# spcl/gms

Hardware: AMD Instinct MI355X
Metric: edges-intersected/sec + achieved HBM GB/s, RMAT-26 triangle count @1/2/4/8 GPU (higher is better)
Workload: dtype int32 ids / uint64 counts

## Files before the change

### gms_amd/csrc/hip/device_graph.hip

```cpp
#include "device_graph.hpp"

#include <algorithm>
#include <mutex>
#include <array>
#include <chrono>
#include <cstdio>
#include <cstdlib>
#include <cstring>
#include <memory>
#include <new>
#include <random>

#include <rocprim/device/device_radix_sort.hpp>
#include <rocprim/device/device_scan.hpp>
#include <rocprim/device/device_segmented_radix_sort.hpp>
#include <rocprim/iterator/transform_iterator.hpp>

#include "../host/gmsx_internal.hpp"
#include "../host/tc_core_plan.hpp"
#include "kc4_mfma.hpp"

namespace gmsx {

Ctx &ctx() {
// ... 599 lines not shown
__global__ void k_ledge_fill(int64_t first, int64_t end, const int32_t *__restrict__ order, const int64_t *__restrict__ hoff, const int64_t *__restrict__ toff,
                             const int32_t *__restrict__ tadj, const int32_t *__restrict__ tsplit, const int32_t *__restrict__ dplus,
                             int32_t core, const int64_t *__restrict__ ebeg, int nparts, int part, uint4 *__restrict__ ledge) {
    const int64_t pos = first + int64_t(blockIdx.x) * blockDim.x + threadIdx.x;
    if (pos >= end) return;
    const int32_t u = order[pos];
    if (u < core) return;
    const int64_t hb = hoff[u], tb = toff[u];
    const int tl = int(toff[u + 1] - tb);
    const unsigned long long hu = (unsigned long long)hb | ((unsigned long long)(hoff[u + 1] - hb) << 40);
    int64_t e = ebeg[pos - first];
    for (int i = tsplit[u]; i < tl; ++i) {
        const int32_t v = tadj[tb + i];
        if (dplus[v] >= kHeavy) continue;
        if (nparts <= 1 || shard_of(e, nparts) == part) {
            const unsigned long long tu = (unsigned long long)tb | ((unsigned long long)i << 40);
            const unsigned long long hv = (unsigned long long)hoff[v] | ((unsigned long long)(hoff[v + 1] - hoff[v]) << 40);
            const unsigned long long tv = (unsigned long long)toff[v] | ((unsigned long long)(toff[v + 1] - toff[v]) << 40);
            const int64_t slot = nparts <= 1 ? e : e / nparts;
            ledge[2 * slot] = make_uint4(uint32_t(hu), uint32_t(hu >> 32), uint32_t(tu), uint32_t(tu >> 32));
            ledge[2 * slot + 1] = make_uint4(uint32_t(hv), uint32_t(hv >> 32), uint32_t(tv), uint32_t(tv >> 32));
        }
        ++e;
    }
}

__device__ __forceinline__ uint32_t cut_hub_units(const uint32_t *__restrict__ spool, unsigned long long d, int below, int32_t v) {
    const uint32_t units = uint32_t(d) & 0x3fffffu, form = (uint32_t(d) >> 22) & 3u;
    if (form == kFormList) return min(units, uint32_t(below + 7) / 8u);
    if (form == kFormBitset) return min(units, uint32_t(v + 127) / 128u);
    const uint4 *row = reinterpret_cast<const uint4 *>(spool) + (d >> 24);
    uint32_t lo = 0, hi = units;
    while (lo < hi) {
        const uint32_t mid = (lo + hi) >> 1;
        if (int32_t(row[mid].x & 0xffffu) < v) lo = mid + 1; else hi = mid;
    }
    return lo;
}
__device__ __forceinline__ uint32_t cut_tail_units(const uint32_t *__restrict__ tpool, unsigned long long d, int below, int32_t v) {
    const uint32_t units = uint32_t(d) & 0x3fffffu, form = (uint32_t(d) >> 22) & 3u;
    if (form != kFormDelta) return min(units, uint32_t(below + 3) / 4u);
    const uint4 *row = reinterpret_cast<const uint4 *>(tpool) + (d >> 24);
    uint32_t lo = 0, hi = units;
    while (lo < hi) {
        const uint32_t mid = (lo + hi) >> 1;
        if (int32_t(row[mid].x) < v) lo = mid + 1; else hi = mid;
// ... 160 lines not shown
        *p = nullptr;
        return GMSX_ERR_DEVICE_MEM;
    }
    if (hipMalloc(reinterpret_cast<void **>(p), bytes) != hipSuccess) {
        (void)hipGetLastError();
        *p = nullptr;
        return GMSX_ERR_DEVICE_MEM;
    }
    if (g) g->device_bytes += int64_t(bytes);
    return GMSX_OK;
}

struct DevGuard {
    void *p;
    ~DevGuard() { (void)hipFree(p); }
};

static void free_tc(gmsx_graph *g) {
    auto drop = [](auto *&p) {
        (void)hipFree(p);
        p = nullptr;
    };
    drop(g->tsplit); drop(g->srow); drop(g->srow2); drop(g->ksplit); drop(g->spool); drop(g->trow); drop(g->htask.lo); drop(g->htask.hi); drop(g->ttask.lo); drop(g->ttask.hi); drop(g->hitem); drop(g->titem); drop(g->tunits);
    drop(g->ledge); drop(g->tpool); drop(g->shard_hitem); drop(g->shard_titem); drop(g->core_bits);
    g->tc_core = 0;
    g->shard_idx_part = g->shard_idx_nparts = -1;
    g->device_bytes -= g->tc_bytes;
    g->tc_bytes = 0;
    g->tc_ready = false;
    g->htask_entries = g->ttask_entries = g->hitems = g->titems = g->inline_hentries = g->inline_tentries = 0;
    g->n_ledge = g->ledge_total = 0;
    g->task_reverse = g->inline_units = g->spool_units = g->tpool_units = 0;
    g->stats_part = g->stats_nparts = -1;
}

static void free_graph(gmsx_graph *g) {
    if (!g) return;
    (void)hipFree(g->off);
    (void)hipFree(g->adj);
    (void)hipFree(g->newid);
    (void)hipFree(g->oldid);
    (void)hipFree(g->hoff);
    (void)hipFree(g->hadj);
    (void)hipFree(g->toff);
    (void)hipFree(g->tadj);
    (void)hipFree(g->bmoff);
    (void)hipFree(g->bmpool);
    (void)hipFree(g->tsplit);
    (void)hipFree(g->srow);
    (void)hipFree(g->srow2);
    (void)hipFree(g->ksplit);
    (void)hipFree(g->spool);
    (void)hipFree(g->trow);
    (void)hipFree(g->htask.lo);
    (void)hipFree(g->htask.hi);
    (void)hipFree(g->ttask.lo);
    (void)hipFree(g->ttask.hi);
    (void)hipFree(g->hitem);
    (void)hipFree(g->titem);
    (void)hipFree(g->tunits);
    (void)hipFree(g->shard_hitem);
    (void)hipFree(g->shard_titem);
    (void)hipFree(g->ledge);
    (void)hipFree(g->core_bits);
    (void)hipFree(g->tpool);
    (void)hipFree(g->dplus);
    (void)hipFree(g->order);
    (void)hipFree(g->kc_rel);
    (void)hipFree(g->kc_aoff);
    (void)hipFree(g->kc_arena);
    (void)hipFree(g->kc_rec);
    (void)hipFree(g->kc_item);
    (void)hipFree(g->kc_relt);
    (void)hipFree(g->kc_rect);
    (void)hipFree(g->kc_itemt);
    (void)hipFree(g->scratch);
    (void)hipFree(g->acc);
    delete g;
}

int exclusive_scan_i64(const int64_t *in, int64_t *out, int64_t count, hipStream_t s) {
    size_t tmp_bytes = 0;
    GMSX_HIP(rocprim::exclusive_scan(nullptr, tmp_bytes, in, out, int64_t(0), size_t(count), rocprim::plus<int64_t>(), s));
    void *tmp = nullptr;
    GMSX_HIP(hipMalloc(&tmp, tmp_bytes ? tmp_bytes : 8));
    DevGuard g_tmp{tmp};
// ... 503 lines not shown
        inline_t_base = big_units + small_units;
        g->tpool_units = inline_t_base + inline_t_units;
        if (g->tpool_units >= (int64_t(1) << 40)) return GMSX_ERR_DEVICE_MEM;
        if (int rc = dmalloc(&g->trow, n, g)) return rc;
        if (int rc = dmalloc(&g->tpool, (g->tpool_units + kPoolSlack) * 4, g)) return rc;
        GMSX_HIP(hipMemsetD32Async(reinterpret_cast<hipDeviceptr_t>(g->tpool), int(0xFFFFFFFEu), size_t(g->tpool_units + kPoolSlack) * 4, s));
        if (n > 0)
            hipLaunchKernelGGL(k_trow_fill, dim3(unsigned((n + 255) / 256)), dim3(256), 0, s, n, g->toff, g->tadj, uoff, soff, real, form, g->trow, g->tpool);
        GMSX_HIP(hipStreamSynchronize(s));
    }

    pt.mark("tail stream rows");
    if (n_work > 0) {
        GMSX_HIP(hipMemsetAsync(inl_h, 0, size_t(n + 1) * sizeof(unsigned long long), s));
        GMSX_HIP(hipMemsetAsync(inl_t, 0, size_t(n + 1) * sizeof(unsigned long long), s));
        hipLaunchKernelGGL(k_inline_rows<true>, dim3(grid_for_waves(n_work)), dim3(256), 0, s, int64_t(0), n_work, g->order, g->hoff, g->hadj, g->toff,
                           g->tadj, g->dplus, g->inline_limit, g->inline_first, g->tc_core, opos, g->shard_nparts, g->shard_part, inl_h, inl_t, ihoff, itoff, inline_h_base, reinterpret_cast<uint16_t *>(g->spool),
                           inline_t_base, reinterpret_cast<int32_t *>(g->tpool));
    }
    pt.mark("inline rows fill");
    {
        const int64_t nl = n_work - n_heavy;
        g->n_ledge = g->ledge_total = 0;
        if (nl > 0) {
            int64_t *ecnt = nullptr, *ebeg = nullptr;
            if (int rc = dmalloc(&ecnt, nl + 1, nullptr)) return rc;
            DevGuard g_ec{ecnt};
            if (int rc = dmalloc(&ebeg, nl + 1, nullptr)) return rc;
            DevGuard g_eb{ebeg};
            hipLaunchKernelGGL(k_ledge_count, dim3(unsigned(nl / 256 + 1)), dim3(256), 0, s, n_heavy, n_work, g->order, g->toff, g->tadj, g->tsplit, g->dplus, g->tc_core, ecnt);
            if (int rc = exclusive_scan_i64(ecnt, ebeg, nl + 1, s)) return rc;
            GMSX_HIP(hipMemcpy(&g->ledge_total, ebeg + nl, sizeof(int64_t), hipMemcpyDeviceToHost));
            const int np = g->shard_nparts > 1 ? g->shard_nparts : 1, pp = g->shard_nparts > 1 ? g->shard_part : 0;
            {
                const int64_t full = g->ledge_total / np, rem = g->ledge_total % np;
                g->n_ledge = np <= 1 ? g->ledge_total : full + (((full & 1) ? np - 1 - pp : pp) < rem ? 1 : 0);
            }
            if (int rc = dmalloc(&g->ledge, 2 * g->n_ledge + 2, g)) return rc;
            hipLaunchKernelGGL(k_ledge_fill, dim3(unsigned(nl / 256 + 1)), dim3(256), 0, s, n_heavy, n_work, g->order, g->hoff, g->toff, g->tadj, g->tsplit, g->dplus, g->tc_core, ebeg,
                               np, pp, g->ledge);
            GMSX_HIP(hipStreamSynchronize(s));
        }
    }
    pt.mark("light pivot list");
    {
        int two_sided = 1;
        if (const char *e = opt("TC_TWO_SIDED")) two_sided = std::atoi(e) != 0;
// ... 404 lines not shown
```

### gms_amd/csrc/hip/device_graph.hpp

```cpp
#pragma once
#include <hip/hip_runtime.h>

#include <cstdint>

#include "gmsx.h"
#include "gmsx_internal.hpp"

#if !defined(GMSX_DEV_HOOKS) &&                                                                                                               \
    (defined(GMSX_KC_NO_PROBE) || defined(GMSX_KC_NO_HITS) || defined(GMSX_KC_NO_TAIL) || defined(GMSX_KC_NO_INNER) || defined(GMSX_KC_CELLS_ONLY) ||   \
     defined(GMSX_KC_NO_ROWS) || defined(GMSX_KC_BUILD_ONLY) || defined(GMSX_KC_NO_SLAB_CALL) || defined(GMSX_KC_NO_PAIRS) || defined(GMSX_KC_SLAB_ROW_SCAN) || \
     defined(GMSX_BK_AB) || defined(GMSX_BK_NO_HIT_ATOMICS) || defined(GMSX_BK_STATS) || defined(GMSX_TC_NO_PROBE) || defined(GMSX_TC_STAGING_ONLY))
#error "A/B switches need -DGMSX_DEV_HOOKS (tools/ab_lib.sh sets it); the default build of libgmsx.so carries none of them"
#endif

struct __attribute__((aligned(64))) gmsx_tc_item {
    uint64_t bc;
    uint64_t cont;
    int32_t pivot;
    int32_t pos;
    uint32_t kind;
    uint16_t fbeg[4];
    uint32_t reserved[7];
};
static_assert(sizeof(gmsx_tc_item) == 64, "work item record = one 64-byte line");
// ... 27 lines not shown
    int32_t *tadj = nullptr;
    int64_t *bmoff = nullptr;
    uint32_t *bmpool = nullptr;
    int32_t dense_limit = 0;
    int32_t bitset_limit = 0;
    unsigned long long *srow = nullptr;
    unsigned long long *srow2 = nullptr;
    int32_t *ksplit = nullptr;
    uint32_t *spool = nullptr;
    int64_t spool_units = 0;
    TaskList htask{nullptr, nullptr, false};
    TaskList ttask{nullptr, nullptr, true};
    int64_t htask_entries = 0, ttask_entries = 0;
    struct gmsx_tc_item *hitem = nullptr, *titem = nullptr;
    int64_t hitems = 0, titems = 0;
    int64_t inline_hentries = 0, inline_tentries = 0;
    mutable struct gmsx_tc_item *shard_hitem = nullptr, *shard_titem = nullptr;
    mutable int64_t shard_hitems = 0, shard_titems = 0;
    mutable int shard_idx_part = -1, shard_idx_nparts = -1;
    int32_t *tunits = nullptr;
    int64_t task_reverse = 0;
    uint4 *ledge = nullptr;
    int64_t n_ledge = 0, ledge_total = 0;
    uint32_t *core_bits = nullptr;
    int32_t tc_core = 0;
    mutable int core_bytes_k = -1, core_bytes_part = -1, core_bytes_nparts = -1;
    mutable uint64_t core_bytes = 0;
    int tc_hot_windows = 0;
    uint32_t tc_window_units = 1;
    int tc_hot_min = 0;
    int inline_first = 64;
    int32_t inline_limit = 0;
    int64_t inline_units = 0;
    unsigned long long *trow = nullptr;
    uint32_t *tpool = nullptr;
    int64_t tpool_units = 0;
    int32_t *tsplit = nullptr;
    int64_t dense_rows = 0, bmpool_words = 0;
    bool rows_sorted = false;
    int32_t *dplus = nullptr;
    int32_t *order = nullptr;
    int64_t hub_entries = 0, tail_entries = 0;
    int32_t max_dplus = 0;
    int32_t max_deg = 0;
    mutable bool kc_rev_tried = false;
    mutable uint32_t *kc_rel = nullptr;
// ... 59 lines not shown
__host__ __device__ inline int tail_class(const TcClasses &cc, unsigned long long d) {
    return cc.tail_base() + (((uint32_t(d) >> 22) & 3u) == 2u ? kLenClasses : 0) + length_class(uint32_t(d) & 0x3fffffu);
}
__host__ __device__ inline void hub_phase_range(const TcClasses &cc, const uint32_t *c, int64_t len, int ph, int64_t *b, int64_t *e) {
    int64_t start = 0;
    for (int q = 0;; ++q) {
        const int64_t end = q < cc.hot_windows ? int64_t(c[(q + 1) * kHubClasses]) : len;
        const bool own = q == cc.hot_windows || end - start >= cc.hot_min;
        if (q == ph) {
            *b = start;
            *e = own ? end : start;
            return;
        }
        if (own) start = end;
    }
}
__host__ __device__ inline int shard_of(int64_t pos, int nparts) {
    const int j = int(pos % nparts);
    return ((pos / nparts) & 1) ? nparts - 1 - j : j;
}
static constexpr int kHeavy = 64;
static constexpr int kDeltaIds = 14;

__host__ __device__ inline int64_t bitset_words(int32_t v) { return ((int64_t(v) + 31) / 32 + 3) & ~int64_t(3); }

struct Ctx {
    int device = -1;
    hipStream_t stream = nullptr;
    hipStream_t own_stream = nullptr;
    hipEvent_t ev[4] = {nullptr, nullptr, nullptr, nullptr};
    hipStream_t side[2] = {nullptr, nullptr};
    hipEvent_t ev_fork = nullptr, ev_join[2] = {nullptr, nullptr};
    int compute_units = 0;
};
Ctx &ctx();
int ensure_init();
int kclique_vertex_counts(const gmsx_graph *g, unsigned long long *d_counts, gmsx_stats *st);
int count_dplus_ge(const gmsx_graph *g, int32_t threshold, int64_t *out);
int exclusive_scan_i64(const int64_t *in, int64_t *out, int64_t count, hipStream_t s);
int ensure_tc(const gmsx_graph *g);
int ensure_tc_shard(const gmsx_graph *g, int part, int nparts);
int tc_shard_items(const gmsx_graph *g, int part, int nparts);
int tc_vertex_counts_device(const gmsx_graph *g, unsigned long long *d_counts, gmsx_stats *st);
int tc_full_partial(const gmsx_graph *g, int part, int nparts, uint64_t *partial, gmsx_stats *st);

__device__ __forceinline__ int uni32(int x) { return __builtin_amdgcn_readfirstlane(x); }
// ... 19 lines not shown
```

### gms_amd/csrc/hip/tc.hip

```cpp
#include "device_graph.hpp"
#include "kc4_mfma.hpp"
#include "../host/tc_core_plan.hpp"

#include <algorithm>
#include <type_traits>
#include <rocprim/device/device_radix_sort.hpp>
#include <rocprim/device/device_reduce.hpp>
#include <rocprim/device/device_reduce_by_key.hpp>
#include <cstdio>
#include <cstdlib>
#include <cstring>

namespace gmsx {

static constexpr int kAccSlots = 64;
static constexpr int kAccStride = 16;

struct __attribute__((packed, aligned(4))) u4u { uint32_t x, y, z, w; };

__device__ __forceinline__ int64_t readlane64(int64_t x, int l) {
    const uint32_t lo = __builtin_amdgcn_readlane(uint32_t(uint64_t(x)), l);
    const uint32_t hi = __builtin_amdgcn_readlane(uint32_t(uint64_t(x) >> 32), l);
    return int64_t((uint64_t(hi) << 32) | lo);
}
// ... 614 lines not shown
            for (int ka = 0; ka < 4; ++ka) {
                if (ka >= nat) break;
                const int ia = sub + 16 * ka;
                const uint32_t a = ia < tlu ? rows.at[ka] : 0xFFFFFFFFu;
                bool m = false;
#pragma unroll
                for (int kb = 0; kb < 4; ++kb) {
                    if (kb >= nbt) break;
                    const int ib = sub + 16 * kb;
                    const uint32_t x = ib < tlv ? rows.bt[kb] : 0xFFFFFFFEu;
                    m |= row_has(a, x);
                }
                c += m ? 1u : 0u;
            }
            total += c;
            rec = rec_n;
            rows = rows_n;
            rec_n = rec_nn;
        }
    }
    block_add(total, red, lane, wave, tid, acc);
}

__global__ __launch_bounds__(1024) void k_tc_core(const uint32_t *__restrict__ bits, int WS, int K, int nb, int nblk, int part, int nparts,
                                                  unsigned long long *__restrict__ acc) {
    __shared__ unsigned long long red[16];
    auto lane_id = [] { return int(__builtin_amdgcn_mbcnt_hi(~0u, __builtin_amdgcn_mbcnt_lo(~0u, 0u))); };
    const int wave = uni32(int(threadIdx.x) >> 6);
    const int x = blockIdx.x & 7, y = blockIdx.x >> 3, Y = int(gridDim.x) >> 3;
    const int Q = 16 * Y, q = y * 16 + wave;
    const int ns = (nblk - part + nparts - 1) / nparts;
    uint32_t cnt = 0;
    for (int j = 0;; ++j) {
        const int sidx = (8 * j + ((j & 1) ? 7 - x : x)) * Q + q;
        if (sidx >= ns) break;
        const int t = sidx * nparts + part;
        int c = int((__builtin_sqrtf(8.0f * float(t) + 1.0f) - 1.0f) * 0.5f);
        while (c * (c + 1) / 2 > t) --c;
        while ((c + 1) * (c + 2) / 2 <= t) ++c;
        const int bj = nb - 1 - c, bi = bj + (t - c * (c + 1) / 2);
        int lane = lane_id();
        asm volatile("" : "+v"(lane));
        cnt += Kc4mBlock<2>::run(bits, WS, K, bi, bj, lane);
    }
    const int lane = lane_id();
    unsigned long long total = cnt;
    for (int sft = 32; sft > 0; sft >>= 1) total += __shfl_down(total, sft);
    if (lane == 0) red[wave] = total;
    __syncthreads();
    if (wave == 0 && lane == 0) {
        unsigned long long t = 0;
        for (int w = 0; w < 16; ++w) t += red[w];
        if (t) atomicAdd(&acc[(blockIdx.x & (kAccSlots - 1)) * kAccStride], t);
    }
}

__global__ __launch_bounds__(256) void k_tc_stats(const int64_t *__restrict__ hoff, const uint16_t *__restrict__ hadj,
                                                  const int64_t *__restrict__ toff, const int32_t *__restrict__ tadj,
                                                  const int32_t *__restrict__ dplus, const int32_t *__restrict__ order,
                                                  const int32_t *__restrict__ tunits, int32_t inline_limit, int inline_first, int32_t core, int64_t end, int nparts, int part,
                                                  unsigned long long *__restrict__ out) {
    const int lane = threadIdx.x & 63;
    const int64_t wave0 = (int64_t(blockIdx.x) * blockDim.x + threadIdx.x) >> 6;
    const int64_t nwaves = (int64_t(gridDim.x) * blockDim.x) >> 6;
    unsigned long long units = 0, probes = 0, bytes = 0;
    for (int64_t pos = wave0; pos < end; pos += nwaves) {
        if (nparts > 1 && shard_of(pos, nparts) != part) continue;
        const int32_t u = order[pos];
        const int du = dplus[u];
        if (du >= kHeavy) {
            if (lane == 0) units += (unsigned long long)tunits[pos];
            if (u < core) {
                if (lane == 0) units += (unsigned long long)du;
                continue;
            }
            const int hl = min(int(hoff[u + 1] - hoff[u]), inline_first), tl = min(int(toff[u + 1] - toff[u]), inline_first - hl);
            int32_t v = -1;
            if (lane < hl) {
                const uint32_t x = hadj[hoff[u] + lane];
                if (x != 0xFFFFu) v = int32_t(x);
            } else if (lane - hl < tl) v = tadj[toff[u] + lane - hl];
            if (v >= 0 && lane > 0 && (v < inline_limit || dplus[v] >= kHeavy)) ++units;
            continue;
        }
        const int hl = int(hoff[u + 1] - hoff[u]);
        if (lane == 0) units += (unsigned long long)du;
        if (du < 2 || u < core) continue;
        for (int64_t j = toff[u] + lane; j < toff[u + 1]; j += 64) {
            const int32_t v = tadj[j];
            if (v < inline_limit || dplus[v] >= kHeavy) continue;
            const unsigned long long hv = (unsigned long long)(hoff[v + 1] - hoff[v]), tv = (unsigned long long)(toff[v + 1] - toff[v]);
            bytes += 32ull + 2ull * hl + 4ull * (unsigned long long)(j - toff[u]) + 2ull * hv + 4ull * tv;
            probes += hv + tv;
        }
    }
    for (int s = 32; s > 0; s >>= 1) {
        units += __shfl_down(units, s);
        probes += __shfl_down(probes, s);
        bytes += __shfl_down(bytes, s);
    }
    if (lane == 0) {
        if (units) atomicAdd(&out[0], units);
        if (probes) atomicAdd(&out[1], probes);
        if (bytes) atomicAdd(&out[2], bytes);
    }
}
__global__ __launch_bounds__(256) void k_tc_item_stats(const int64_t *__restrict__ coff, int bytes_per_id, int tail, const TaskList task,
                                                       const gmsx_tc_item *__restrict__ items, int64_t n_items, int nparts, int part,
                                                       unsigned long long *__restrict__ out) {
    const int lane = threadIdx.x & 63;
    const int64_t wave0 = (int64_t(blockIdx.x) * blockDim.x + threadIdx.x) >> 6;
    const int64_t nwaves = (int64_t(gridDim.x) * blockDim.x) >> 6;
    unsigned long long probes = 0, bytes = 0;
    auto slots = [tail](unsigned long long d) -> unsigned long long {
        const unsigned long long n = d & 0x3fffffull, f = (d >> 22) & 3ull;
// ... 1 lines not shown
    };
    for (int64_t q = wave0; q < n_items; q += nwaves) {
        const gmsx_tc_item &it = items[q];
        if (nparts > 1 && shard_of(it.pos, nparts) != part) continue;
        const int ne = int(it.bc >> 40);
        const int64_t b = int64_t(it.bc & 0xffffffffffull);
        if (lane == 0) bytes += (unsigned long long)bytes_per_id * (unsigned long long)(coff[it.pivot + 1] - coff[it.pivot]);
        for (int i = lane; i < ne; i += 64) {
            const unsigned long long d = task.get(b + i);
            bytes += 6ull + 16ull * (d & 0x3fffffull);
            probes += slots(d);
        }
    }
    for (int s = 32; s > 0; s >>= 1) {
        probes += __shfl_down(probes, s);
        bytes += __shfl_down(bytes, s);
    }
    if (lane == 0) {
        if (probes) atomicAdd(&out[1], probes);
        if (bytes) atomicAdd(&out[2], bytes);
    }
}

__global__ __launch_bounds__(256) void k_tc_breakdown(const int64_t *__restrict__ hoff, const int64_t *__restrict__ toff, const int32_t *__restrict__ tadj,
                                                      const int32_t *__restrict__ dplus, const int32_t *__restrict__ order,
                                                      const TaskList htask, const gmsx_tc_item *__restrict__ hitem, int64_t hitems,
                                                      const TaskList ttask, const gmsx_tc_item *__restrict__ titem, int64_t titems,
                                                      int32_t inline_limit, int32_t core, int64_t first_light, int64_t end_light,
                                                      unsigned long long *__restrict__ out) {
    const int lane = threadIdx.x & 63;
    const int64_t wave0 = (int64_t(blockIdx.x) * blockDim.x + threadIdx.x) >> 6;
    const int64_t nwaves = (int64_t(gridDim.x) * blockDim.x) >> 6;
    unsigned long long c[15] = {0, 0, 0, 0, 0, 0, 0, 0, 0, 0, 0, 0, 0, 0, 0};
    for (int64_t q = wave0; q < hitems + titems; q += nwaves) {
        const bool tail = q >= hitems;
        const gmsx_tc_item &it = tail ? titem[q - hitems] : hitem[q];
        const TaskList task = tail ? ttask : htask;
        const int ne = int(it.bc >> 40);
        const int64_t b0 = int64_t(it.bc & 0xffffffffffull);
        if (lane == 0) {
            c[6] += tail ? 4ull * (unsigned long long)(toff[it.pivot + 1] - toff[it.pivot]) : 2ull * (unsigned long long)(hoff[it.pivot + 1] - hoff[it.pivot]);
            c[11] += (unsigned long long)ne;
            c[13] += 1;
        }
        for (int i = lane; i < ne; i += 64) {
            const unsigned long long d = task.get(b0 + i);
            const unsigned long long db = 16ull * (d & 0x3fffffull);
            const int fd = int((d >> 22) & 3);
            if (tail) c[fd == kFormDelta ? 4 : 3] += db;
            else c[fd == kFormList ? 0 : fd == kFormBitset ? 1 : 2] += db;
            c[5] += 6;
        }
    }
    for (int64_t pos = first_light + wave0; pos < end_light; pos += nwaves) {
        const int32_t u = order[pos];
        if (u < core) continue;
        const int64_t tb0 = toff[u], te = toff[u + 1];
        const unsigned long long hl = (unsigned long long)(hoff[u + 1] - hoff[u]);
        for (int64_t j = tb0 + lane; j < te; j += 64) {
            const int32_t v = tadj[j];
            if (v < inline_limit || dplus[v] >= kHeavy) continue;
            c[8] += 2ull * (unsigned long long)(hoff[v + 1] - hoff[v]);
            c[9] += 4ull * (unsigned long long)(toff[v + 1] - toff[v]);
            c[10] += 32ull + 2ull * hl + 4ull * (unsigned long long)(j - tb0);
            c[14] += 1;
        }
    }
    for (int k = 0; k < 15; ++k) {
        unsigned long long x = c[k];
        for (int s = 32; s > 0; s >>= 1) x += __shfl_down(x, s);
        if (lane == 0 && x) atomicAdd(&out[k], x);
    }
}

__device__ __forceinline__ int hist_bin(unsigned long long units) {
    if (units <= 16) return int(units) - 1;
    int b = 16;
    for (unsigned long long lim = 32; units > lim && b < 23; lim <<= 1) ++b;
    return b;
}
__global__ __launch_bounds__(256) void k_tc_comember_keys(const TaskList htask, const gmsx_tc_item *__restrict__ hitem, int64_t hitems, int batch,
                                                         unsigned long long *__restrict__ keys, uint32_t *__restrict__ vals, unsigned long long *__restrict__ sums) {
    unsigned long long ents = 0, units = 0;
    for (int64_t i = blockIdx.x; i < hitems; i += gridDim.x) {
        const gmsx_tc_item it = hitem[i];
        const unsigned long long first = it.bc & 0xffffffffffull;
        const int n = int(it.bc >> 40);
        const unsigned long long b = (unsigned long long)(it.pos / batch) << 40;
// ... 169 lines not shown
    const char *only = std::getenv("GMSX_TC_ONLY");
    if (only) {
        if (std::strcmp(only, "hub") != 0) n_hitems = 0;
        if (std::strcmp(only, "tail") != 0) n_titems = 0;
    }
#else
    const char *only = nullptr;
#endif
    Ctx &c = ctx();
    hipStream_t s = c.stream;
    unsigned long long *acc = g->acc;
    static_assert(kAccSlots * kAccStride + 16 <= kAccWords, "gmsx_graph::acc too small");
    unsigned int *qhead = reinterpret_cast<unsigned int *>(acc + kAccSlots * kAccStride + 4);
    static_assert((kQueueStride + 1) * sizeof(unsigned int) <= 12 * sizeof(unsigned long long), "queue heads past gmsx_graph::acc");
    GMSX_HIP(hipEventRecord(c.ev[0], s));
    GMSX_HIP(hipMemsetAsync(acc, 0, sizeof(unsigned long long) * kAccWords, s));
    GMSX_HIP(hipEventRecord(c.ev[1], s));

    int launches = 0;
    const int cus = c.compute_units > 0 ? c.compute_units : 256;
    const int64_t cap_blocks = int64_t(cus) * 16;
    const bool run_light = !only || std::strcmp(only, "light") == 0;
    const bool strided = nparts > 1 && g->shard_nparts == 1;
    const int64_t cnt_light = [&]() -> int64_t {
        if (!run_light) return 0;
        if (!strided) return g->n_ledge;
        const int64_t full = g->n_ledge / nparts, rem = g->n_ledge % nparts;
        return full + (((full & 1) ? nparts - 1 - part : part) < rem ? 1 : 0);
    }();
    const int overlap = [] { const char *e = opt("TC_OVERLAP"); return e ? std::atoi(e) : 0; }();
    const int persist = [] { const char *e = opt("TC_PERSIST"); return e ? std::atoi(e) : 1; }();
    const bool sides = overlap && c.side[0] && c.side[1];
    struct Join {
        Ctx &c;
        hipStream_t s;
        bool armed[2] = {false, false};
        ~Join() {
            for (int i = 0; i < 2; ++i)
                if (armed[i] && hipEventRecord(c.ev_join[i], c.side[i]) == hipSuccess) (void)hipStreamWaitEvent(s, c.ev_join[i], 0);
        }
    } join{c, s};
    const bool side_light = sides && cnt_light > 0 && n_hitems + n_titems > 0;
    const bool side_tail = sides && !persist && n_hitems > 0 && n_titems > 0;
    if (side_light || side_tail) GMSX_HIP(hipEventRecord(c.ev_fork, s));
    if (side_tail) {
        GMSX_HIP(hipStreamWaitEvent(c.side[0], c.ev_fork, 0));
        join.armed[0] = true;
    }
    if (side_light) {
        GMSX_HIP(hipStreamWaitEvent(c.side[1], c.ev_fork, 0));
        join.armed[1] = true;
    }
// ... 11 lines not shown
        const int wgs_env = [] { const char *e = opt("TC_ITEM_WGS"); return e ? std::atoi(e) : 0; }();
        auto grid = [&](int64_t n, int wgs) {
            return unsigned(std::max<int64_t>(1, std::min<int64_t>((n + kGrab - 1) / kGrab, int64_t(cus) * (wgs_env > 0 ? wgs_env : wgs))));
        };
        if (n_hitems > 0) {
            hipLaunchKernelGGL(k_tc_items<false>, dim3(grid(n_hitems, GMSX_TC_HUB_MIN_WAVES)), dim3(256), 0, s, g->hadj, g->tadj, g->spool, g->htask, hitem, int(n_hitems), qhead, acc);
            ++launches;
        }
        if (n_titems > 0) {
            hipLaunchKernelGGL(k_tc_items<true>, dim3(grid(n_titems, GMSX_TC_TAIL_MIN_WAVES)), dim3(256), 0, s, g->hadj, g->tadj, g->tpool, g->ttask, titem, int(n_titems),
                               qhead + kQueueStride, acc);
            ++launches;
        }
    } else {
        if (n_hitems > 0) {
            hipLaunchKernelGGL(k_tc_block, dim3(unsigned(n_hitems)), dim3(256), 0, s, g->hoff, g->hadj, g->spool, g->htask, hitem, acc);
            ++launches;
        }
        if (n_titems > 0) {
            hipLaunchKernelGGL(k_tc_tail, dim3(unsigned(n_titems)), dim3(256), 0, side_tail ? c.side[0] : s, g->toff, g->tadj, g->tpool, g->ttask, titem, acc);
            ++launches;
        }
    }
    if (cnt_light > 0) {
        const int64_t blocks = std::min<int64_t>((cnt_light + 15) / 16, int64_t(cus) * 8);
        hipLaunchKernelGGL(k_tc_light, dim3(unsigned(blocks)), dim3(256), 0, side_light ? c.side[1] : s, g->hadj, g->tadj, g->ledge, strided ? nparts : 1,
                           strided ? part : 0, cnt_light, acc);
        ++launches;
    }
    for (int i = 0; i < 2; ++i)
        if (join.armed[i]) {
            join.armed[i] = false;
            GMSX_HIP(hipEventRecord(c.ev_join[i], c.side[i]));
            GMSX_HIP(hipStreamWaitEvent(s, c.ev_join[i], 0));
        }
    GMSX_HIP(hipEventRecord(c.ev[2], s));
    GMSX_HIP(hipGetLastError());

    const bool need_stats = st && !(g->stats_part == part && g->stats_nparts == nparts);
    if (need_stats) {
        if (g->n > 0) {
            const int64_t blocks = std::min<int64_t>((g->n + 3) / 4, cap_blocks);
            hipLaunchKernelGGL(k_tc_stats, dim3(unsigned(blocks)), dim3(256), 0, s, g->hoff, g->hadj, g->toff, g->tadj, g->dplus, g->order,
                               g->tunits, g->inline_limit, g->inline_first, g->tc_core, g->n, nparts, part, acc + kAccSlots * kAccStride);
        }
        if (g->hitems > 0)
            hipLaunchKernelGGL(k_tc_item_stats, dim3(unsigned(std::min<int64_t>((g->hitems + 3) / 4, cap_blocks))), dim3(256), 0, s, g->hoff, 2, 0, g->htask, g->hitem,
                               g->hitems, nparts, part, acc + kAccSlots * kAccStride);
        if (g->titems > 0)
            hipLaunchKernelGGL(k_tc_item_stats, dim3(unsigned(std::min<int64_t>((g->titems + 3) / 4, cap_blocks))), dim3(256), 0, s, g->toff, 4, 1, g->ttask, g->titem,
                               g->titems, nparts, part, acc + kAccSlots * kAccStride);
    }
    unsigned long long host[kAccSlots * kAccStride + 3];
    GMSX_HIP(hipMemcpyAsync(host, acc, sizeof(host), hipMemcpyDeviceToHost, s));
    GMSX_HIP(hipStreamSynchronize(s));
    unsigned long long total = 0;
    for (int i = 0; i < kAccSlots; ++i) total += host[i * kAccStride];
    *partial = total;
    if (st) {
        float ms_setup = 0.f, ms_kernel = 0.f;
        GMSX_HIP(hipEventElapsedTime(&ms_setup, c.ev[0], c.ev[1]));
        GMSX_HIP(hipEventElapsedTime(&ms_kernel, c.ev[1], c.ev[2]));
        st->kernel_ms = ms_kernel;
        st->setup_ms = ms_setup;
        if (need_stats) {
            g->stats_part = part;
            g->stats_nparts = nparts;
// ... 15 lines not shown

using namespace gmsx;

extern "C" {

int gmsx_tc_divisor(int algo) { return algo == GMSX_TC_FULL ? 3 : 1; }

int gmsx_tc_stream_breakdown(const gmsx_graph *g, uint64_t *out21) {
    return gmsx::guard([&]() -> int {
        if (!g || !out21) return GMSX_ERR_INVALID;
        if (int rc = ensure_init()) return rc;
        if (int rc = ensure_tc(g)) return rc;
        hipStream_t s = ctx().stream;
        std::memset(out21, 0, 21 * sizeof(uint64_t));
        if (g->n == 0) return GMSX_OK;
        int64_t n_block = 0, n_work = 0;
        if (int rc = count_dplus_ge(g, kHeavy, &n_block)) return rc;
        if (int rc = count_dplus_ge(g, 2, &n_work)) return rc;
        unsigned long long *acc = nullptr;
        GMSX_HIP(hipMalloc(reinterpret_cast<void **>(&acc), 21 * 8));
        struct Guard { void *p; ~Guard() { (void)hipFree(p); } } g1{acc};
        GMSX_HIP(hipMemsetAsync(acc, 0, 21 * 8, s));
        const int cus = ctx().compute_units > 0 ? ctx().compute_units : 256;
        hipLaunchKernelGGL(k_tc_breakdown, dim3(unsigned(cus * 16)), dim3(256), 0, s, g->hoff, g->toff, g->tadj, g->dplus, g->order, g->htask,
                           g->hitem, g->hitems, g->ttask, g->titem, g->titems, g->inline_limit, g->tc_core, n_block, n_work, acc);
        GMSX_HIP(hipMemcpyAsync(out21, acc, 21 * 8, hipMemcpyDeviceToHost, s));
        GMSX_HIP(hipStreamSynchronize(s));
        GMSX_HIP(hipGetLastError());
        out21[7] = uint64_t(g->inline_units) * 16ull;
        out21[12] = uint64_t(g->inline_hentries + g->inline_tentries);
        out21[15] = core_bytes_of(g, 0, 1);
        out21[16] = uint64_t(g->tc_core);
        return GMSX_OK;
    });
}

int gmsx_tc_row_histogram(const gmsx_graph *g, uint64_t *out256) {
    return gmsx::guard([&]() -> int {
        uint64_t *out248 = out256;
        if (!g || !out248) return GMSX_ERR_INVALID;
        if (int rc = ensure_init()) return rc;
        if (int rc = ensure_tc(g)) return rc;
        hipStream_t s = ctx().stream;
        std::memset(out248, 0, 256 * sizeof(uint64_t));
        if (g->n == 0) return GMSX_OK;
        unsigned long long *acc = nullptr;
        GMSX_HIP(hipMalloc(reinterpret_cast<void **>(&acc), 256 * 8));
        struct Guard { void *p; ~Guard() { (void)hipFree(p); } } g1{acc};
// ... 90 lines not shown
```

### gms_amd/csrc/host/loader.cpp

```cpp
#include "gmsx_internal.hpp"

#include <fcntl.h>
#include <sys/mman.h>
#include <sys/stat.h>
#include <unistd.h>

#include <algorithm>
#ifdef _OPENMP
#include <parallel/algorithm>
#endif
#include <atomic>
#include <cerrno>
#include <cmath>
#include <cstdio>
#include <cstdlib>
#include <cstring>
#include <ctime>
#include <fstream>
#include <limits>
#include <memory>
#include <new>
#include <random>
#include <sstream>
#include <string>
// ... 631 lines not shown
void parallel_memcpy(void *dst, const void *src, size_t bytes) {
#ifdef _OPENMP
#pragma omp parallel
    {
        const size_t nt = size_t(omp_get_num_threads()), t = size_t(omp_get_thread_num());
        const size_t per = ((bytes + nt - 1) / nt + 4095) & ~size_t(4095), lo = std::min(bytes, per * t), hi = std::min(bytes, lo + per);
        if (hi > lo) std::memcpy(static_cast<char *>(dst) + lo, static_cast<const char *>(src) + lo, hi - lo);
    }
#else
    std::memcpy(dst, src, bytes);
#endif
}
namespace {
struct Option {
    const char *name;
    char value[32];
    bool set;
};
Option g_options[] = {
    {"TIMING", "", false}, {"MEM_TRACE", "", false}, {"BK_VERBOSE", "", false},
    {"INLINE_LIMIT", "", false}, {"TC_INLINE_FIRST", "", false}, {"TC_DELTA", "", false}, {"TC_DELTA_PCT", "", false}, {"TC_GAP12", "", false},
    {"TC_HYBRID", "", false}, {"TC_TAIL_DELTA", "", false}, {"TC_TWO_SIDED", "", false}, {"TC_HOT_WINDOWS", "", false}, {"TC_HOT_KB", "", false},
    {"TC_HOT_MIN", "", false}, {"TC_TEST_MAX_UNITS", "", false}, {"TC_KEEP_ROWS", "", false}, {"TC_MEM_LIMIT_MB", "", false}, {"TC_OVERLAP", "", false},
    {"TC_PERSIST", "", false}, {"TC_ITEM_WGS", "", false}, {"TC_CORE", "", false}, {"SORT_CHUNK", "", false}, {"UPLOAD_STAGED", "", false}, {"INIT_LAZY", "", false},
    {"KC_SLAB_MB", "", false}, {"KC_MAXD", "", false}, {"KC_STREAMS", "", false}, {"KC_PIPE_ALL", "", false}, {"KC_STREAM_BUILD", "", false},
    {"KC_REVERSE", "", false}, {"KC_REV_MIN", "", false}, {"KC_REV_FACTOR", "", false}, {"KC_REV_TAIL", "", false}, {"KC_REV_TAIL_MIN", "", false}, {"KC_REV_GW", "", false}, {"KC_TRI", "", false}, {"KC_MFMA", "", false}, {"KC_POOL_MB", "", false},
    {"BK_MAXC", "", false}, {"BK_ARENA_MB", "", false}, {"BK_GROUPS", "", false}, {"BK_SMALL_P", "", false}, {"BK_SMALL_P_GROUPS", "", false},
    {"BK_BUDGET", "", false}, {"BK_BUDGET0", "", false}, {"BK_RESUME_GRAB", "", false}, {"BK_SPLIT_BUILD", "", false}, {"BK_TINY_ROOTS", "", false},
    {"BK_TINY_BESIDE", "", false},
    {"BK_LIST_ARENA_MB", "", false},
    {"KCSTAR_SLAB_MB", "", false},
    {"CORE_WG_FRONTIER", "", false},
    {"COLOR_WG_FRONTIER", "", false},
    {"TRUSS_WG_FRONTIER", "", false},
    {"LP_LDS_MAXN", "", false}, {"LP_SLAB_MB", "", false},
};
Option *find_option(const char *name) {
    if (!name) return nullptr;
    for (Option &o : g_options)
        if (std::strcmp(o.name, name) == 0) return &o;
    return nullptr;
}
}

const char *opt(const char *name) {
    const Option *o = find_option(name);
    return o && o->set ? o->value : nullptr;
// ... 242 lines not shown
```

Before: 16.10 billion.

## Pack light edge pairs into contiguous size-classed blocks for triangle counting

Replaces the indirect light-edge descriptors (offsets into hub and tail adjacency pools) with pre-materialised, padded blocks that hold both endpoints' hub and tail id lists, grouped into six size classes. A new templated kernel per class streams each block with coalesced loads into LDS and does fixed-depth branchless binary searches, prefetching the next block while it computes. This targets scattered gathers and variable-length loops in the light path. In exchange it costs extra preprocessing, duplicated adjacency storage with padding overhead, and six launches instead of one.

```diff
diff --git a/gms_amd/csrc/hip/device_graph.hip b/gms_amd/csrc/hip/device_graph.hip
--- a/gms_amd/csrc/hip/device_graph.hip
+++ b/gms_amd/csrc/hip/device_graph.hip
@@ -645,6 +645,84 @@
             ledge[2 * slot + 1] = make_uint4(uint32_t(hv), uint32_t(hv >> 32), uint32_t(tv), uint32_t(tv >> 32));
         }
         ++e;
+    }
+}
+
+__global__ void k_lpack_count(int64_t first, int64_t end, const int32_t *__restrict__ order, const int64_t *__restrict__ hoff, const uint16_t *__restrict__ hadj,
+                              const int64_t *__restrict__ toff, const int32_t *__restrict__ tadj, const int32_t *__restrict__ tsplit, const int32_t *__restrict__ dplus,
+                              int32_t core, int64_t *__restrict__ cnt) {
+    const int64_t p = int64_t(blockIdx.x) * blockDim.x + threadIdx.x, nl = end - first;
+    if (p >= nl) return;
+    int64_t c[kLightClasses];
+#pragma unroll
+    for (int k = 0; k < kLightClasses; ++k) c[k] = 0;
+    const int32_t u = order[first + p];
+    if (u >= core) {
+        const int64_t tb = toff[u];
+        const int tl = int(toff[u + 1] - tb), ah = light_hub_ids(hoff, hadj, u);
+        for (int i = tsplit[u]; i < tl; ++i) {
+            const int32_t v = tadj[tb + i];
+            if (dplus[v] >= kHeavy) continue;
+            const int cls = light_class(ah, i, light_hub_ids(hoff, hadj, v), int(toff[v + 1] - toff[v]));
+#pragma unroll
+            for (int k = 0; k < kLightClasses; ++k) c[k] += cls == k ? 1 : 0;
+        }
+    }
+#pragma unroll
+    for (int k = 0; k < kLightClasses; ++k) cnt[int64_t(k) * nl + p] = c[k];
+}
+struct LpackPlan {
+    int64_t class_beg[kLightClasses];
+    int64_t unit_base[kLightClasses];
+};
+__device__ __forceinline__ uint4 lpack_hub_unit(const uint16_t *__restrict__ row, int len, int q) {
+    uint32_t w[4];
+#pragma unroll
+    for (int j = 0; j < 4; ++j) {
+        const int i = 8 * q + 2 * j;
+        const uint32_t lo = i < len ? row[i] : 0xFFFFu, hi = i + 1 < len ? row[i + 1] : 0xFFFFu;
+        w[j] = lo | (hi << 16);
+    }
+    return make_uint4(w[0], w[1], w[2], w[3]);
+}
+__device__ __forceinline__ uint4 lpack_tail_unit(const int32_t *__restrict__ row, int len, int q, uint32_t filler) {
+    uint32_t w[4];
+#pragma unroll
+    for (int j = 0; j < 4; ++j) w[j] = 4 * q + j < len ? uint32_t(row[4 * q + j]) : filler;
+    return make_uint4(w[0], w[1], w[2], w[3]);
+}
+__global__ void k_lpack_fill(int64_t first, int64_t end, const int32_t *__restrict__ order, const int64_t *__restrict__ hoff, const uint16_t *__restrict__ hadj,
+                             const int64_t *__restrict__ toff, const int32_t *__restrict__ tadj, const int32_t *__restrict__ tsplit, const int32_t *__restrict__ dplus,
+                             int32_t core, const int64_t *__restrict__ beg, const LpackPlan plan, int nparts, int part, uint4 *__restrict__ lpack) {
+    const int64_t p = int64_t(blockIdx.x) * blockDim.x + threadIdx.x, nl = end - first;
+    if (p >= nl) return;
+    const int32_t u = order[first + p];
+    if (u < core) return;
+    int64_t next[kLightClasses];
+#pragma unroll
+    for (int k = 0; k < kLightClasses; ++k) next[k] = beg[int64_t(k) * nl + p] - plan.class_beg[k];
+    const int64_t hb = hoff[u], tb = toff[u];
+    const int tl = int(toff[u + 1] - tb), ah = light_hub_ids(hoff, hadj, u);
+    for (int i = tsplit[u]; i < tl; ++i) {
+        const int32_t v = tadj[tb + i];
+        if (dplus[v] >= kHeavy) continue;
+        const int64_t hv = hoff[v], tv = toff[v];
+        const int bh = light_hub_ids(hoff, hadj, v), bt = int(toff[v + 1] - tv);
+        const int cls = light_class(ah, i, bh, bt);
+        int64_t k = 0, base = 0;
+#pragma unroll
+        for (int c = 0; c < kLightClasses; ++c)
+            if (cls == c) {
+                k = next[c]++;
+                base = plan.unit_base[c];
+            }
+        if (nparts > 1 && shard_of(k, nparts) != part) continue;
+        const LightShape sh = light_shape(cls);
+        uint4 *blk = lpack + base + (nparts <= 1 ? k : k / nparts) * sh.stride();
+        for (int q = 0; q < sh.ah; ++q) *blk++ = lpack_hub_unit(hadj + hb, ah, q);
+        for (int q = 0; q < sh.at; ++q) *blk++ = lpack_tail_unit(tadj + tb, i, q, 0xFFFFFFFFu);
+        for (int q = 0; q < sh.bh; ++q) *blk++ = lpack_hub_unit(hadj + hv, bh, q);
+        for (int q = 0; q < sh.bt; ++q) *blk++ = lpack_tail_unit(tadj + tv, bt, q, 0xFFFFFFFEu);
     }
 }
 
@@ -851,7 +929,7 @@
         p = nullptr;
     };
     drop(g->tsplit); drop(g->srow); drop(g->srow2); drop(g->ksplit); drop(g->spool); drop(g->trow); drop(g->htask.lo); drop(g->htask.hi); drop(g->ttask.lo); drop(g->ttask.hi); drop(g->hitem); drop(g->titem); drop(g->tunits);
-    drop(g->ledge); drop(g->tpool); drop(g->shard_hitem); drop(g->shard_titem); drop(g->core_bits);
+    drop(g->ledge); drop(g->lpack); drop(g->tpool); drop(g->shard_hitem); drop(g->shard_titem); drop(g->core_bits);
     g->tc_core = 0;
     g->shard_idx_part = g->shard_idx_nparts = -1;
     g->device_bytes -= g->tc_bytes;
@@ -859,6 +937,7 @@
     g->tc_ready = false;
     g->htask_entries = g->ttask_entries = g->hitems = g->titems = g->inline_hentries = g->inline_tentries = 0;
     g->n_ledge = g->ledge_total = 0;
+    for (int c = 0; c < 8; ++c) g->lpack_base[c] = g->lpack_n[c] = g->lpack_total[c] = 0;
     g->task_reverse = g->inline_units = g->spool_units = g->tpool_units = 0;
     g->stats_part = g->stats_nparts = -1;
 }
@@ -891,6 +970,7 @@
     (void)hipFree(g->shard_hitem);
     (void)hipFree(g->shard_titem);
     (void)hipFree(g->ledge);
+    (void)hipFree(g->lpack);
     (void)hipFree(g->core_bits);
     (void)hipFree(g->tpool);
     (void)hipFree(g->dplus);
@@ -1440,7 +1520,47 @@
     {
         const int64_t nl = n_work - n_heavy;
         g->n_ledge = g->ledge_total = 0;
-        if (nl > 0) {
+        g->light_packed = opt_int("TC_LIGHT_PACKED", 1) != 0;
+        for (int c = 0; c < 8; ++c) g->lpack_base[c] = g->lpack_n[c] = g->lpack_total[c] = 0;
+        if (nl > 0 && g->light_packed) {
+            int64_t *ecnt = nullptr, *ebeg = nullptr;
+            const int64_t cells = int64_t(kLightClasses) * nl;
+            if (int rc = dmalloc(&ecnt, cells + 1, nullptr)) return rc;
+            DevGuard g_ec{ecnt};
+            if (int rc = dmalloc(&ebeg, cells + 1, nullptr)) return rc;
+            DevGuard g_eb{ebeg};
+            GMSX_HIP(hipMemsetAsync(ecnt + cells, 0, sizeof(int64_t), s));
+            hipLaunchKernelGGL(k_lpack_count, dim3(unsigned(nl / 256 + 1)), dim3(256), 0, s, n_heavy, n_work, g->order, g->hoff, g->hadj, g->toff, g->tadj, g->tsplit, g->dplus,
+                               g->tc_core, ecnt);
+            if (int rc = exclusive_scan_i64(ecnt, ebeg, cells + 1, s)) return rc;
+            const int np = g->shard_nparts > 1 ? g->shard_nparts : 1, pp = g->shard_nparts > 1 ? g->shard_part : 0;
+            LpackPlan plan{};
+            int64_t units = 0;
+            for (int c = 0; c < kLightClasses; ++c) {
+                int64_t b[2] = {0, 0};
+                GMSX_HIP(hipMemcpy(&b[0], ebeg + int64_t(c) * nl, sizeof(int64_t), hipMemcpyDeviceToHost));
+                GMSX_HIP(hipMemcpy(&b[1], ebeg + int64_t(c + 1) * nl, sizeof(int64_t), hipMemcpyDeviceToHost));
+                const int64_t total = b[1] - b[0], full = total / np, rem = total % np;
+                plan.class_beg[c] = b[0];
+                plan.unit_base[c] = units;
+                g->lpack_total[c] = total;
+                g->lpack_n[c] = np <= 1 ? total : full + (((full & 1) ? np - 1 - pp : pp) < rem ? 1 : 0);
+                g->lpack_base[c] = units;
+                units += g->lpack_n[c] * light_shape(c).stride();
+                g->ledge_total += total;
+                g->n_ledge += g->lpack_n[c];
+            }
+            if (opt("MEM_TRACE"))
+                for (int c = 0; c < kLightClasses; ++c) {
+                    const LightShape k = light_shape(c);
+                    std::fprintf(stderr, "gmsx light class %d (ids <= %d / %d / %d / %d, %d units): %lld blocks\n", c, 8 * k.ah, 4 * k.at, 8 * k.bh, 4 * k.bt, k.stride(),
+                                 (long long)g->lpack_total[c]);
+                }
+            if (int rc = dmalloc(&g->lpack, units + 1, g)) return rc;
+            hipLaunchKernelGGL(k_lpack_fill, dim3(unsigned(nl / 256 + 1)), dim3(256), 0, s, n_heavy, n_work, g->order, g->hoff, g->hadj, g->toff, g->tadj, g->tsplit, g->dplus,
+                               g->tc_core, ebeg, plan, np, pp, g->lpack);
+            GMSX_HIP(hipStreamSynchronize(s));
+        } else if (nl > 0) {
             int64_t *ecnt = nullptr, *ebeg = nullptr;
             if (int rc = dmalloc(&ecnt, nl + 1, nullptr)) return rc;
             DevGuard g_ec{ecnt};
diff --git a/gms_amd/csrc/hip/device_graph.hpp b/gms_amd/csrc/hip/device_graph.hpp
--- a/gms_amd/csrc/hip/device_graph.hpp
+++ b/gms_amd/csrc/hip/device_graph.hpp
@@ -73,6 +73,11 @@
     int64_t task_reverse = 0;
     uint4 *ledge = nullptr;
     int64_t n_ledge = 0, ledge_total = 0;
+    uint4 *lpack = nullptr;
+    int64_t lpack_base[8] = {0, 0, 0, 0, 0, 0, 0, 0};
+    int64_t lpack_n[8] = {0, 0, 0, 0, 0, 0, 0, 0};
+    int64_t lpack_total[8] = {0, 0, 0, 0, 0, 0, 0, 0};
+    bool light_packed = false;
     uint32_t *core_bits = nullptr;
     int32_t tc_core = 0;
     mutable int core_bytes_k = -1, core_bytes_part = -1, core_bytes_nparts = -1;
@@ -178,6 +183,31 @@
 static constexpr int kHeavy = 64;
 static constexpr int kDeltaIds = 14;
 
+struct LightShape {
+    int ah, at, bh, bt;
+    __host__ __device__ constexpr int stride() const { return ah + at + bh + bt; }
+};
+static constexpr int kLightClasses = 6;
+static_assert(kLightClasses <= 8, "gmsx_graph::lpack_base");
+__host__ __device__ constexpr LightShape light_shape(int c) {
+    return c == 0 ? LightShape{2, 3, 2, 4} : c == 1 ? LightShape{1, 2, 5, 8} : c == 2 ? LightShape{2, 4, 5, 9} : c == 3 ? LightShape{3, 8, 4, 9}
+         : c == 4 ? LightShape{6, 8, 6, 10} : LightShape{8, 16, 8, 16};
+}
+static_assert(kHeavy <= 8 * light_shape(kLightClasses - 1).ah && kHeavy <= 4 * light_shape(kLightClasses - 1).at &&
+              kHeavy <= 8 * light_shape(kLightClasses - 1).bh && kHeavy <= 4 * light_shape(kLightClasses - 1).bt, "the last class must hold every light row");
+static constexpr int kLightMaxUnits = light_shape(kLightClasses - 1).stride();
+__host__ __device__ inline int light_class(int ah, int at, int bh, int bt) {
+    for (int c = 0; c < kLightClasses - 1; ++c) {
+        const LightShape k = light_shape(c);
+        if (ah <= 8 * k.ah && at <= 4 * k.at && bh <= 8 * k.bh && bt <= 4 * k.bt) return c;
+    }
+    return kLightClasses - 1;
+}
+__device__ __forceinline__ int light_hub_ids(const int64_t *__restrict__ hoff, const uint16_t *__restrict__ hadj, int32_t v) {
+    const int64_t b = hoff[v], e = hoff[v + 1];
+    return int(e - b) - ((e > b && hadj[e - 1] == 0xFFFFu) ? 1 : 0);
+}
+
 __host__ __device__ inline int64_t bitset_words(int32_t v) { return ((int64_t(v) + 31) / 32 + 3) & ~int64_t(3); }
 
 struct Ctx {
diff --git a/gms_amd/csrc/hip/tc.hip b/gms_amd/csrc/hip/tc.hip
--- a/gms_amd/csrc/hip/tc.hip
+++ b/gms_amd/csrc/hip/tc.hip
@@ -660,6 +660,72 @@
     block_add(total, red, lane, wave, tid, acc);
 }
 
+template <int N, class T>
+__device__ __forceinline__ bool lds_has(const T *b, uint32_t a) {
+    uint32_t pos = 0;
+#pragma unroll
+    for (int len = N; len > 1; len -= len / 2) pos += uint32_t(b[pos + len / 2 - 1]) < a ? uint32_t(len / 2) : 0u;
+    return uint32_t(b[pos]) == a;
+}
+__device__ __forceinline__ void wave_lds_fence() {
+    __builtin_amdgcn_fence(__ATOMIC_RELEASE, "wavefront");
+    __builtin_amdgcn_wave_barrier();
+    __builtin_amdgcn_fence(__ATOMIC_ACQUIRE, "wavefront");
+}
+template <int C>
+__global__ __launch_bounds__(256) void k_tc_lpack(const uint4 *__restrict__ blocks, int nparts, int part, int64_t count, unsigned long long *__restrict__ acc) {
+    constexpr LightShape K = light_shape(C);
+    constexpr int S = K.stride(), STEPS = (S + 15) / 16;
+    constexpr int AH = 8 * K.ah, AT = 4 * K.at, BH = 8 * K.bh, BT = 4 * K.bt;
+    constexpr int RAH = (AH + 15) / 16, RAT = (AT + 15) / 16;
+    static_assert(2 * RAH <= STEPS * 16 && K.ah + 4 * RAT <= STEPS * 16, "a lane past the end of a part of u reads inside the group's slice");
+    __shared__ uint4 slab[16 * STEPS * 16];
+    __shared__ unsigned long long red[4];
+    const int tid = threadIdx.x, lane = tid & 63, wave = tid >> 6, sub = lane & 15;
+    uint4 *mine = slab + (tid >> 4) * (STEPS * 16);
+    const uint16_t *ah = reinterpret_cast<const uint16_t *>(mine), *bh = reinterpret_cast<const uint16_t *>(mine + K.ah + K.at);
+    const uint32_t *at = reinterpret_cast<const uint32_t *>(mine + K.ah), *bt = reinterpret_cast<const uint32_t *>(mine + K.ah + K.at + K.bh);
+    const int64_t ngroups = int64_t(gridDim.x) * 16, g0 = int64_t(blockIdx.x) * 16 + (tid >> 4);
+    const int64_t trips = (count + ngroups - 1) / ngroups;
+    struct Units {
+        uint4 u[STEPS];
+    };
+    auto load = [&](int64_t t) -> Units {
+        const int64_t k = g0 + t * ngroups;
+        const int64_t kk = k < count ? k : 0;
+        const int64_t e = nparts <= 1 ? kk : kk * nparts + ((kk & 1) ? nparts - 1 - part : part);
+        const uint4 *blk = blocks + e * S;
+        Units r;
+#pragma unroll
+        for (int s = 0; s < STEPS; ++s) r.u[s] = blk[min(sub + 16 * s, S - 1)];
+        return r;
+    };
+    unsigned long long total = 0;
+    if (trips > 0) {
+        Units cur = load(0);
+        for (int64_t t = 0; t < trips; ++t) {
+#pragma unroll
+            for (int s = 0; s < STEPS; ++s) mine[16 * s + sub] = cur.u[s];
+            wave_lds_fence();
+            cur = load(t + 1);
+            uint32_t c = 0;
+#pragma unroll
+            for (int r = 0; r < RAH; ++r) {
+                const uint32_t a = ah[sub + 16 * r];
+                c += (lds_has<BH>(bh, a) && a != 0xFFFFu && (16 * (r + 1) <= AH || sub + 16 * r < AH)) ? 1u : 0u;
+            }
+#pragma unroll
+            for (int r = 0; r < RAT; ++r) {
+                const uint32_t a = (16 * (r + 1) <= AT || sub + 16 * r < AT) ? at[sub + 16 * r] : 0xFFFFFFFFu;
+                c += lds_has<BT>(bt, a) ? 1u : 0u;
+            }
+            wave_lds_fence();
+            total += g0 + t * ngroups < count ? c : 0u;
+        }
+    }
+    block_add(total, red, lane, wave, tid, acc);
+}
+
 __global__ __launch_bounds__(1024) void k_tc_core(const uint32_t *__restrict__ bits, int WS, int K, int nb, int nblk, int part, int nparts,
                                                   unsigned long long *__restrict__ acc) {
     __shared__ unsigned long long red[16];
@@ -696,7 +762,7 @@
 __global__ __launch_bounds__(256) void k_tc_stats(const int64_t *__restrict__ hoff, const uint16_t *__restrict__ hadj,
                                                   const int64_t *__restrict__ toff, const int32_t *__restrict__ tadj,
                                                   const int32_t *__restrict__ dplus, const int32_t *__restrict__ order,
-                                                  const int32_t *__restrict__ tunits, int32_t inline_limit, int inline_first, int32_t core, int64_t end, int nparts, int part,
+                                                  const int32_t *__restrict__ tunits, int32_t inline_limit, int inline_first, int32_t core, int packed, int64_t end, int nparts, int part,
                                                   unsigned long long *__restrict__ out) {
     const int lane = threadIdx.x & 63;
     const int64_t wave0 = (int64_t(blockIdx.x) * blockDim.x + threadIdx.x) >> 6;
@@ -724,11 +790,13 @@
         const int hl = int(hoff[u + 1] - hoff[u]);
         if (lane == 0) units += (unsigned long long)du;
         if (du < 2 || u < core) continue;
+        const int ah = packed ? light_hub_ids(hoff, hadj, u) : 0;
         for (int64_t j = toff[u] + lane; j < toff[u + 1]; j += 64) {
             const int32_t v = tadj[j];
             if (v < inline_limit || dplus[v] >= kHeavy) continue;
             const unsigned long long hv = (unsigned long long)(hoff[v + 1] - hoff[v]), tv = (unsigned long long)(toff[v + 1] - toff[v]);
-            bytes += 32ull + 2ull * hl + 4ull * (unsigned long long)(j - toff[u]) + 2ull * hv + 4ull * tv;
+            if (packed) bytes += 16ull * (unsigned long long)light_shape(light_class(ah, int(j - toff[u]), light_hub_ids(hoff, hadj, v), int(tv))).stride();
+            else bytes += 32ull + 2ull * hl + 4ull * (unsigned long long)(j - toff[u]) + 2ull * hv + 4ull * tv;
             probes += hv + tv;
         }
     }
@@ -776,11 +844,11 @@
     }
 }
 
-__global__ __launch_bounds__(256) void k_tc_breakdown(const int64_t *__restrict__ hoff, const int64_t *__restrict__ toff, const int32_t *__restrict__ tadj,
+__global__ __launch_bounds__(256) void k_tc_breakdown(const int64_t *__restrict__ hoff, const uint16_t *__restrict__ hadj, const int64_t *__restrict__ toff, const int32_t *__restrict__ tadj,
                                                       const int32_t *__restrict__ dplus, const int32_t *__restrict__ order,
                                                       const TaskList htask, const gmsx_tc_item *__restrict__ hitem, int64_t hitems,
                                                       const TaskList ttask, const gmsx_tc_item *__restrict__ titem, int64_t titems,
-                                                      int32_t inline_limit, int32_t core, int64_t first_light, int64_t end_light,
+                                                      int32_t inline_limit, int32_t core, int packed, int64_t first_light, int64_t end_light,
                                                       unsigned long long *__restrict__ out) {
     const int lane = threadIdx.x & 63;
     const int64_t wave0 = (int64_t(blockIdx.x) * blockDim.x + threadIdx.x) >> 6;
@@ -811,13 +879,20 @@
         if (u < core) continue;
         const int64_t tb0 = toff[u], te = toff[u + 1];
         const unsigned long long hl = (unsigned long long)(hoff[u + 1] - hoff[u]);
+        const int ah = packed ? light_hub_ids(hoff, hadj, u) : 0;
         for (int64_t j = tb0 + lane; j < te; j += 64) {
             const int32_t v = tadj[j];
             if (v < inline_limit || dplus[v] >= kHeavy) continue;
+            c[14] += 1;
+            if (packed) {
+                const LightShape k = light_shape(light_class(ah, int(j - tb0), light_hub_ids(hoff, hadj, v), int(toff[v + 1] - toff[v])));
+                c[8] += 16ull * (unsigned long long)(k.ah + k.bh);
+                c[9] += 16ull * (unsigned long long)(k.at + k.bt);
+                continue;
+            }
             c[8] += 2ull * (unsigned long long)(hoff[v + 1] - hoff[v]);
             c[9] += 4ull * (unsigned long long)(toff[v + 1] - toff[v]);
             c[10] += 32ull + 2ull * hl + 4ull * (unsigned long long)(j - tb0);
-            c[14] += 1;
         }
     }
     for (int k = 0; k < 15; ++k) {
@@ -1033,12 +1108,15 @@
     const int64_t cap_blocks = int64_t(cus) * 16;
     const bool run_light = !only || std::strcmp(only, "light") == 0;
     const bool strided = nparts > 1 && g->shard_nparts == 1;
-    const int64_t cnt_light = [&]() -> int64_t {
+    auto light_share = [&](int64_t held) -> int64_t {
         if (!run_light) return 0;
-        if (!strided) return g->n_ledge;
-        const int64_t full = g->n_ledge / nparts, rem = g->n_ledge % nparts;
+        if (!strided) return held;
+        const int64_t full = held / nparts, rem = held % nparts;
         return full + (((full & 1) ? nparts - 1 - part : part) < rem ? 1 : 0);
-    }();
+    };
+    int64_t cnt_class[kLightClasses], cnt_light = 0;
+    for (int k = 0; k < kLightClasses; ++k) cnt_light += cnt_class[k] = g->light_packed ? light_share(g->lpack_n[k]) : 0;
+    if (!g->light_packed) cnt_light = light_share(g->n_ledge);
     const int overlap = [] { const char *e = opt("TC_OVERLAP"); return e ? std::atoi(e) : 0; }();
     const int persist = [] { const char *e = opt("TC_PERSIST"); return e ? std::atoi(e) : 1; }();
     const bool sides = overlap && c.side[0] && c.side[1];
@@ -1096,7 +1174,22 @@
             ++launches;
         }
     }
-    if (cnt_light > 0) {
+    if (g->light_packed) {
+        auto launch = [&](auto kernel, int k) {
+            if (cnt_class[k] <= 0) return;
+            const int64_t blocks = std::min<int64_t>((cnt_class[k] + 15) / 16, int64_t(cus) * 8);
+            hipLaunchKernelGGL(kernel, dim3(unsigned(blocks)), dim3(256), 0, side_light ? c.side[1] : s, g->lpack + g->lpack_base[k], strided ? nparts : 1, strided ? part : 0,
+                               cnt_class[k], acc);
+            ++launches;
+        };
+        static_assert(kLightClasses == 6, "one instance per class");
+        launch(k_tc_lpack<0>, 0);
+        launch(k_tc_lpack<1>, 1);
+        launch(k_tc_lpack<2>, 2);
+        launch(k_tc_lpack<3>, 3);
+        launch(k_tc_lpack<4>, 4);
+        launch(k_tc_lpack<5>, 5);
+    } else if (cnt_light > 0) {
         const int64_t blocks = std::min<int64_t>((cnt_light + 15) / 16, int64_t(cus) * 8);
         hipLaunchKernelGGL(k_tc_light, dim3(unsigned(blocks)), dim3(256), 0, side_light ? c.side[1] : s, g->hadj, g->tadj, g->ledge, strided ? nparts : 1,
                            strided ? part : 0, cnt_light, acc);
@@ -1116,7 +1209,7 @@
         if (g->n > 0) {
             const int64_t blocks = std::min<int64_t>((g->n + 3) / 4, cap_blocks);
             hipLaunchKernelGGL(k_tc_stats, dim3(unsigned(blocks)), dim3(256), 0, s, g->hoff, g->hadj, g->toff, g->tadj, g->dplus, g->order,
-                               g->tunits, g->inline_limit, g->inline_first, g->tc_core, g->n, nparts, part, acc + kAccSlots * kAccStride);
+                               g->tunits, g->inline_limit, g->inline_first, g->tc_core, g->light_packed ? 1 : 0, g->n, nparts, part, acc + kAccSlots * kAccStride);
         }
         if (g->hitems > 0)
             hipLaunchKernelGGL(k_tc_item_stats, dim3(unsigned(std::min<int64_t>((g->hitems + 3) / 4, cap_blocks))), dim3(256), 0, s, g->hoff, 2, 0, g->htask, g->hitem,
@@ -1178,8 +1271,8 @@
         struct Guard { void *p; ~Guard() { (void)hipFree(p); } } g1{acc};
         GMSX_HIP(hipMemsetAsync(acc, 0, 21 * 8, s));
         const int cus = ctx().compute_units > 0 ? ctx().compute_units : 256;
-        hipLaunchKernelGGL(k_tc_breakdown, dim3(unsigned(cus * 16)), dim3(256), 0, s, g->hoff, g->toff, g->tadj, g->dplus, g->order, g->htask,
-                           g->hitem, g->hitems, g->ttask, g->titem, g->titems, g->inline_limit, g->tc_core, n_block, n_work, acc);
+        hipLaunchKernelGGL(k_tc_breakdown, dim3(unsigned(cus * 16)), dim3(256), 0, s, g->hoff, g->hadj, g->toff, g->tadj, g->dplus, g->order, g->htask,
+                           g->hitem, g->hitems, g->ttask, g->titem, g->titems, g->inline_limit, g->tc_core, g->light_packed ? 1 : 0, n_block, n_work, acc);
         GMSX_HIP(hipMemcpyAsync(out21, acc, 21 * 8, hipMemcpyDeviceToHost, s));
         GMSX_HIP(hipStreamSynchronize(s));
         GMSX_HIP(hipGetLastError());
diff --git a/gms_amd/csrc/host/loader.cpp b/gms_amd/csrc/host/loader.cpp
--- a/gms_amd/csrc/host/loader.cpp
+++ b/gms_amd/csrc/host/loader.cpp
@@ -677,7 +677,7 @@
     {"INLINE_LIMIT", "", false}, {"TC_INLINE_FIRST", "", false}, {"TC_DELTA", "", false}, {"TC_DELTA_PCT", "", false}, {"TC_GAP12", "", false},
     {"TC_HYBRID", "", false}, {"TC_TAIL_DELTA", "", false}, {"TC_TWO_SIDED", "", false}, {"TC_HOT_WINDOWS", "", false}, {"TC_HOT_KB", "", false},
     {"TC_HOT_MIN", "", false}, {"TC_TEST_MAX_UNITS", "", false}, {"TC_KEEP_ROWS", "", false}, {"TC_MEM_LIMIT_MB", "", false}, {"TC_OVERLAP", "", false},
-    {"TC_PERSIST", "", false}, {"TC_ITEM_WGS", "", false}, {"TC_CORE", "", false}, {"SORT_CHUNK", "", false}, {"UPLOAD_STAGED", "", false}, {"INIT_LAZY", "", false},
+    {"TC_PERSIST", "", false}, {"TC_ITEM_WGS", "", false}, {"TC_CORE", "", false}, {"TC_LIGHT_PACKED", "", false}, {"SORT_CHUNK", "", false}, {"UPLOAD_STAGED", "", false}, {"INIT_LAZY", "", false},
     {"KC_SLAB_MB", "", false}, {"KC_MAXD", "", false}, {"KC_STREAMS", "", false}, {"KC_PIPE_ALL", "", false}, {"KC_STREAM_BUILD", "", false},
     {"KC_REVERSE", "", false}, {"KC_REV_MIN", "", false}, {"KC_REV_FACTOR", "", false}, {"KC_REV_TAIL", "", false}, {"KC_REV_TAIL_MIN", "", false}, {"KC_REV_GW", "", false}, {"KC_TRI", "", false}, {"KC_MFMA", "", false}, {"KC_POOL_MB", "", false},
     {"BK_MAXC", "", false}, {"BK_ARENA_MB", "", false}, {"BK_GROUPS", "", false}, {"BK_SMALL_P", "", false}, {"BK_SMALL_P_GROUPS", "", false},
```

After: 16.66 billion (median of 6 runs). +3.4%, better.
